# kunalchelani/EdgeGaussians

Measured on AMD Instinct MI355X. Metric: train-step Gaussians*views/sec, higher is better.
Workload: dtype f32; 1 GPU; config2: 100000 Gaussians (5:1 anisotropic, scale 0.004, opacity U(0.05,0.9)), 50 views @512x512, real poses of scan 00004926 (intrinsics 800->512); synthetic wireframe edge maps, loss whole/bg_edge_ratio 4:1; n_gaussians=100000, views=50, width=512, height=512, poses=real poses of scan 00004926 (intrinsics 800->512); synthetic wireframe edge maps, largest_tile_population=2957, gaussian_row_order=morton, binning=segmented, steps_per_native_enqueue=50, forward_mode=chained (exact transmittance stop resolved inside the forward kernel), parallelism=single GPU

## Files before the change

edgegaussians_amd/build.py:

```python
from __future__ import annotations

import os
import shutil
import subprocess
import sys
from concurrent.futures import ThreadPoolExecutor

HERE = os.path.dirname(os.path.abspath(__file__))
CSRC = os.path.join(HERE, "csrc")
LIB = os.path.join(HERE, "libedgegs.so")
OBJ = os.path.join(HERE, "csrc", "_obj")
SOURCES = ["project.hip", "binning.hip", "composite.hip", "composite_wide.hip", "composite_wave.hip", "densify.hip", "knn.hip", "step.hip", "dp.hip", "operator.hip", "backward_fused.hip", "cams.hip", "edges.hip", "sh.hip", "packed.hip", "viewmat_grad.hip", "tiles.hip", "functional.hip", "indices.hip", "adam_sparse.hip", "strategy.hip"]
FLAGS = ["--offload-arch=gfx950", "-O3", "-std=c++17", "-fPIC", "-munsafe-fp-atomics", "-fno-slp-vectorize",
         "-Wall", "-Wno-unused-function"]
FLAGS += os.environ.get("EG_EXTRA_HIPCC_FLAGS", "").split()


def _hipcc() -> str:
    for c in (os.environ.get("HIPCC"), shutil.which("hipcc"), "/opt/rocm/bin/hipcc"):
        if c and os.path.exists(c):
            return c
    raise RuntimeError("hipcc not found: libedgegs.so cannot be built")


STAMP = os.path.join(OBJ, "flags.txt")


def _stale() -> bool:
    if not os.path.exists(LIB):
        return True
    if not os.path.exists(STAMP) or open(STAMP).read() != " ".join(FLAGS):
        return True
    t = os.path.getmtime(LIB)
    deps = [os.path.join(CSRC, f) for f in SOURCES + ["common.h", "composite.h", "project_dev.h", "footprint_dev.h", "wide_dev.h"]]
    deps.append(os.path.join(HERE, "..", "include", "edgegs.h"))
    return any(os.path.getmtime(d) > t for d in deps)


def build(force: bool = False, verbose: bool = True) -> str:
    if not force and not _stale():
        return LIB
    hipcc = _hipcc()
    os.makedirs(OBJ, exist_ok=True)

    def compile_one(src: str) -> str:
        obj = os.path.join(OBJ, src.replace(".hip", ".o"))
        cmd = [hipcc, *FLAGS, "-c", os.path.join(CSRC, src), "-o", obj]
        r = subprocess.run(cmd, capture_output=True, text=True)
        if r.returncode != 0:
            raise RuntimeError(f"hipcc failed on {src}:\n{r.stderr}")
        if verbose and r.stderr.strip():
            print(r.stderr, file=sys.stderr)
        return obj

    with ThreadPoolExecutor(max_workers=len(SOURCES)) as ex:
        objs = list(ex.map(compile_one, SOURCES))
    tmp = LIB + ".tmp"
    r = subprocess.run([hipcc, "--offload-arch=gfx950", "-shared", "-fPIC", *objs, "-ldl", "-o", tmp],
                       capture_output=True, text=True)
    if r.returncode != 0:
        raise RuntimeError(f"link failed:\n{r.stderr}")
    os.replace(tmp, LIB)
    with open(STAMP, "w") as f:
        f.write(" ".join(FLAGS))
    if verbose:
        print(f"built {LIB}")
    return LIB


if __name__ == "__main__":
    build(force="--force" in sys.argv)
```

edgegaussians_amd/csrc/backward_fused.hip:

```cpp
#include "common.h"
#include "footprint_dev.h"
#include "project_dev.h"

namespace eg {

constexpr int kBFWaves = 8;
constexpr int kBFGauss = 8 * kBFWaves;
constexpr int kBFTouched = 512;
static_assert(kBFTouched + 1 <= 8 * kBFWaves * 12, "the touched list reuses the footprint sizes' storage");

struct FusedBwdArgs {
  float *means, *quats, *scales, *opacities;
  const float *viewmat, *K, *next_viewmat, *next_K;
  int N, width, height;
  float eps2d;
  uint32_t flags;
  float4 *splat;
  const StopRec *gtstop;
  float *g2d;
  float *absgrads, *am, *av;
  AdamK hyper;
  int *cursor; int seg_cap; unsigned long long *keys;
  float *loss_part, *loss_out;
};

struct TailLds {
  int *hist, *base, *touched, *ntouched;
};
#ifdef EG_BF_PROF
#define EG_BF_STAMP2(k_)                                                           \
  do {                                                                             \
    if (prof_rec) {                                                                \
      asm volatile("s_waitcnt vmcnt(0) lgkmcnt(0)" ::: "memory");                  \
      const unsigned long long t_ = __builtin_amdgcn_s_memrealtime();              \
      if (lane == 0) prof_rec[k_] = t_;                                            \
    }                                                                              \
  } while (0)
#else
#define EG_BF_STAMP2(k_) do {} while (0)
#endif
__device__ __forceinline__ void gaussian_tail(const FusedBwdArgs &a, const int g, const int lane, Raw raw,
                                              float (&mm)[11], float (&vv)[11], const float4 ga, const float4 gb,
                                              const TailLds lds, unsigned long long *prof_rec) {
  const int width = a.width, height = a.height, N = a.N;
  const int tw = (width + kTile - 1) / kTile, th = (height + kTile - 1) / kTile, T = tw * th;
  const float4 *splat = a.splat;
  int *s_hist = lds.hist, *s_base = lds.base, *s_touched = lds.touched;
  int &s_ntouched = *lds.ntouched;
  const bool alive = g < N;
  if (alive) {
    raw = load_raw(a.means, a.quats, a.scales, a.opacities, g);
    const int radius = __float_as_int(splat[2 * g + 1].w);
    const size_t oM = 0, oS = 3 * (size_t)N, oQ = 6 * (size_t)N, oO = 10 * (size_t)N;
    const Cam cam = load_cam(a.viewmat, a.K);
    Grads gr;
#pragma unroll
    for (int k = 0; k < 3; ++k) gr.mean[k] = gr.scale[k] = 0.f;
#pragma unroll
    for (int k = 0; k < 4; ++k) gr.quat[k] = 0.f;
    gr.opac = 0.f;
    if (radius > 0) {
      const float ag = a.absgrads ? a.absgrads[g] : 0.f;
      Fwd f;
      forward_geom(cam, raw, width, height, -3.0e38f, 3.0e38f, a.eps2d, a.flags, f);
      backward_geom(cam, f, a.eps2d, a.flags, ga, gb, false, 0.f, 0.f, gr);
      if (a.absgrads) a.absgrads[g] = ag + sqrtf(ga.z * ga.z + ga.w * ga.w);
    }
    EG_BF_STAMP2(3);
#pragma unroll
    for (int k = 0; k < 3; ++k) {
      mm[k] = a.am[oM + 3 * g + k]; vv[k] = a.av[oM + 3 * g + k];
      mm[3 + k] = a.am[oS + 3 * g + k]; vv[3 + k] = a.av[oS + 3 * g + k];
    }
#pragma unroll
    for (int k = 0; k < 4; ++k) { mm[6 + k] = a.am[oQ + 4 * g + k]; vv[6 + k] = a.av[oQ + 4 * g + k]; }
    mm[10] = a.am[oO + g]; vv[10] = a.av[oO + g];
#pragma unroll
    for (int k = 0; k < 3; ++k) {
      adam1(raw.m[k], gr.mean[k], mm[k], vv[k], 0, a.hyper);
      a.means[3 * g + k] = raw.m[k]; a.am[oM + 3 * g + k] = mm[k]; a.av[oM + 3 * g + k] = vv[k];
    }
#pragma unroll
    for (int k = 0; k < 3; ++k) {
      adam1(raw.s[k], gr.scale[k], mm[3 + k], vv[3 + k], 1, a.hyper);
      a.scales[3 * g + k] = raw.s[k]; a.am[oS + 3 * g + k] = mm[3 + k]; a.av[oS + 3 * g + k] = vv[3 + k];
    }
#pragma unroll
    for (int k = 0; k < 4; ++k) {
      adam1(raw.q[k], gr.quat[k], mm[6 + k], vv[6 + k], 2, a.hyper);
      a.quats[4 * g + k] = raw.q[k]; a.am[oQ + 4 * g + k] = mm[6 + k]; a.av[oQ + 4 * g + k] = vv[6 + k];
    }
    adam1(raw.o, gr.opac, mm[10], vv[10], 3, a.hyper);
    a.opacities[g] = raw.o; a.am[oO + g] = mm[10]; a.av[oO + g] = vv[10];
  }

  EG_BF_STAMP2(4);
  const Cam ncam = load_cam(a.next_viewmat, a.next_K);
  Fwd f;
  int radius = 0;
  if (alive && forward_geom(ncam, raw, width, height, 0.01f, 1e10f, 0.3f, a.flags, f))
    radius = radius_of(f, width, height, 0.f);
  const bool aa = a.flags & EG_FLAG_ANTIALIASED;
  float4 s0 = make_float4(0.f, 0.f, 0.f, 0.f), s1 = s0;
  if (radius > 0) {
    s0 = make_float4(f.u, f.v, f.a, f.b);
    s1 = make_float4(f.c, aa ? f.o * f.comp : f.o, f.z, __int_as_float(radius));
  }
  if (alive) {
    a.splat[2 * g] = s0;
    a.splat[2 * g + 1] = s1;
  }
  int x0 = 0, y0 = 0, x1 = 0, y1 = 0;
  if (radius > 0) tile_box_tight(s0.x, s0.y, radius, s0.z, s0.w, s1.x, s1.y, tw, th, x0, y0, x1, y1);
  const int bw = x1 - x0;
  const bool small_box = (y1 - y0) * bw <= 32;
  unsigned mask = 0u;
  {
    int bit = 0;
    for (int ty = y0; ty < y1; ++ty)
      for (int tx = x0; tx < x1; ++tx, ++bit) {
        if (!splat_hits_tile(s0.x, s0.y, s0.z, s0.w, s1.x, s1.y, tx, ty)) continue;
        if (small_box) mask |= 1u << bit;
        const int t = ty * tw + tx;
        if (atomicAdd(&s_hist[t], 1) == 0) {
          const int idx = atomicAdd(&s_ntouched, 1);
          if (idx < kBFTouched) s_touched[idx] = t;
        }
      }
  }
  EG_BF_STAMP2(5);
  __builtin_amdgcn_fence(__ATOMIC_RELEASE, "wavefront");
  __builtin_amdgcn_wave_barrier();
  __builtin_amdgcn_fence(__ATOMIC_ACQUIRE, "wavefront");
  const int nt = s_ntouched;
  if (nt <= kBFTouched) {
    for (int i = lane; i < nt; i += 64) {
      const int t = s_touched[i];
      const int c = s_hist[t];
      s_base[t] = atomicAdd(&a.cursor[t], c);
      s_hist[t] = 0;
    }
  } else {
    for (int t = lane; t < T; t += 64) {
      const int c = s_hist[t];
      if (c) { s_base[t] = atomicAdd(&a.cursor[t], c); s_hist[t] = 0; }
    }
  }
  __builtin_amdgcn_fence(__ATOMIC_RELEASE, "wavefront");
  __builtin_amdgcn_wave_barrier();
  __builtin_amdgcn_fence(__ATOMIC_ACQUIRE, "wavefront");
  EG_BF_STAMP2(6);
  const unsigned long long key = ((unsigned long long)(unsigned)__float_as_int(s1.z) << 32) | (unsigned)g;
  for (int ty = y0; ty < y1; ++ty)
    for (int tx = x0; tx < x1; ++tx) {
      const bool hit = small_box ? ((mask >> ((ty - y0) * bw + (tx - x0))) & 1u) != 0u
                                 : splat_hits_tile(s0.x, s0.y, s0.z, s0.w, s1.x, s1.y, tx, ty);
      if (!hit) continue;
      const int t = ty * tw + tx;
      const int slot = s_base[t] + atomicAdd(&s_hist[t], 1);
      if (slot < a.seg_cap) a.keys[(size_t)t * a.seg_cap + slot] = key;
    }
  EG_BF_STAMP2(7);
}

__global__ void __launch_bounds__(64 * kBFWaves) __attribute__((amdgpu_waves_per_eu(4, 4)))
gaussian_bwd_fused_kernel(const FusedBwdArgs a) {
  extern __shared__ __attribute__((aligned(16))) int s_dyn[];
  __shared__ __attribute__((aligned(16))) int s_walk[kBFGauss * 12];
  __shared__ __attribute__((aligned(16))) float s_g2d[kBFGauss * 8];
  float *red = (float *)s_dyn;
  int *s_touched = s_walk;
  int &s_ntouched = s_walk[kBFTouched];
  const int width = a.width, height = a.height, N = a.N;
  const int tw = (width + kTile - 1) / kTile, th = (height + kTile - 1) / kTile, T = tw * th;
  int *s_hist = s_dyn, *s_base = s_dyn + T;
  const int lane = threadIdx.x & 63, wv = threadIdx.x >> 6;
  const float4 *splat = a.splat;
#ifdef EG_BF_PROF
  unsigned long long *prof_rec = (unsigned long long *)(a.g2d + 8 * (size_t)a.N) + (size_t)blockIdx.x * 16;
#define EG_BF_STAMP(k_)                                                            \
  do {                                                                             \
    if (a.g2d && wv == 0) {                                                        \
      asm volatile("s_waitcnt vmcnt(0) lgkmcnt(0)" ::: "memory");                  \
      const unsigned long long t_ = __builtin_amdgcn_s_memrealtime();              \
      if (lane == 0) prof_rec[k_] = t_;                                            \
    }                                                                              \
  } while (0)
#else
#define EG_BF_STAMP(k_) do {} while (0)
#endif
  EG_BF_STAMP(0);
  const int g2 = blockIdx.x * kBFGauss + lane;
  Raw raw = {};
  float mm[11], vv[11];
#pragma unroll
  for (int k = 0; k < 11; ++k) mm[k] = vv[k] = 0.f;

  if (a.loss_part && blockIdx.x == 0 && wv == 1) {
    float v = a.loss_part[lane];
    if (v != 0.f) a.loss_part[lane] = 0.f;
    v = wave_sum_dpp_f(v);
    if (lane == 63 && v != 0.f) unsafeAtomicAdd(a.loss_out, v);
  }
  const int gbase = blockIdx.x * kBFGauss + wv * 8;
  if (threadIdx.x < kBFGauss) {
    const int hg = blockIdx.x * kBFGauss + (int)threadIdx.x;
    Walk w = walk_of(make_float4(0.f, 0.f, 0.f, 0.f), make_float4(0.f, 0.f, 0.f, 0.f), width, height);
    if (hg < N) w = walk_of(splat[2 * hg], splat[2 * hg + 1], width, height);
    int4 *dst = (int4 *)&s_walk[12 * threadIdx.x];
    dst[0] = make_int4(w.i0, w.fh, w.pw, w.jlo);
    dst[1] = make_int4(w.jhi, w.cells, __float_as_int(w.thr), __float_as_int(w.xoff));
    dst[2] = make_int4(__float_as_int(w.shear), 0, 0, 0);
  }
  __syncthreads();
  if (gbase < N) {
    const __amdgpu_buffer_rsrc_t rec_rsrc =
        __builtin_amdgcn_make_buffer_rsrc((void *)a.gtstop, 0, width * height * (int)sizeof(StopRec), 0x00020000);
    Walk h;
    {
      const int4 *src = (const int4 *)&s_walk[12 * (wv * 8 + (lane >> 3))];
      const int4 p = src[0], q = src[1];
      h.i0 = p.x; h.fh = p.y; h.pw = p.z; h.jlo = p.w; h.jhi = q.x; h.cells = q.y;
      h.thr = __int_as_float(q.z); h.xoff = __int_as_float(q.w); h.shear = __int_as_float(src[2].x);
    }
    int total = h.cells, live = h.cells > 0 ? 1 : 0;
#pragma unroll
    for (int d = 8; d < 64; d <<= 1) {
      total += __shfl_xor(total, d, 64);
      live += __shfl_xor(live, d, 64);
    }
    int h_n = 0, h_first = 0;
    Moments m = {0.f, 0.f, 0.f, 0.f, 0.f, 0.f, 0.f, 0.f};
    float4 s0 = make_float4(0.f, 0.f, 0.f, 0.f), s1 = s0;
    if (total > 0) {
      const float share = (float)(64 - live) * (1.f - 1e-5f) * __builtin_amdgcn_rcpf((float)total);
      h_n = h.cells > 0 ? 1 + (int)((float)h.cells * share) : 0;
      int incl = h_n + (h.cells > 0 ? 1 << 16 : 0);
#pragma unroll
      for (int d = 8; d < 64; d <<= 1) {
        const int up = __shfl_up(incl, d, 64);
        if (lane >= d) incl += up;
      }
      const int slack = 64 - (__builtin_amdgcn_readlane(incl, 63) & 0xffff);
      const int rank = (incl >> 16) - (h.cells > 0 ? 1 : 0);
      h_first = (incl & 0xffff) - h_n + min(rank, slack);
      if (h.cells > 0 && rank < slack) ++h_n;
      int k = 0;
#pragma unroll
      for (int q = 1; q < 8; ++q) k += lane >= __builtin_amdgcn_readlane(h_first, 8 * q);
      const int src = 8 * k;
      const int n = max(__shfl(h_n, src, 64), 1);
      const int r = lane - __shfl(h_first, src, 64);
      const int g = min(gbase + k, N - 1);
      const int cells = r < n ? __shfl(h.cells, src, 64) : 0;
      s0 = splat[2 * g];
      s1 = splat[2 * g + 1];
      const int4 *wk = (const int4 *)&s_walk[12 * (wv * 8 + k)];
      const int4 p = wk[0], q = wk[1];
      const float shear_k = __int_as_float(wk[2].x);
      footprint_walk(s0, s1, g, r, n, p.x, cells > 0 ? p.y : 0, max(p.z, 1), p.w, q.x, __int_as_float(q.z),
                     __int_as_float(q.w), shear_k, width, rec_rsrc, m);
    }
    float *mine = red + wv * 256 + lane * 4;
    const int comp = lane & 7;
    float sum = 0.f;
    *(float4 *)mine = make_float4(s0.z * m.w_x + s0.w * m.w_y, s0.w * m.w_x + s1.x * m.w_y, (2.f / kLog2e) * m.abs_x,
                                  (2.f / kLog2e) * m.abs_y);
    __builtin_amdgcn_fence(__ATOMIC_RELEASE, "wavefront");
    __builtin_amdgcn_wave_barrier();
    __builtin_amdgcn_fence(__ATOMIC_ACQUIRE, "wavefront");
    if (comp < 4)
      for (int t = 0; t < h_n; ++t) sum += red[wv * 256 + (h_first + t) * 4 + comp];
    __builtin_amdgcn_fence(__ATOMIC_RELEASE, "wavefront");
    __builtin_amdgcn_wave_barrier();
    __builtin_amdgcn_fence(__ATOMIC_ACQUIRE, "wavefront");
    *(float4 *)mine = make_float4(0.5f * m.w_xx, m.w_xy, 0.5f * m.w_yy, m.v_o);
    __builtin_amdgcn_fence(__ATOMIC_RELEASE, "wavefront");
    __builtin_amdgcn_wave_barrier();
    __builtin_amdgcn_fence(__ATOMIC_ACQUIRE, "wavefront");
    if (comp >= 4)
      for (int t = 0; t < h_n; ++t) sum += red[wv * 256 + (h_first + t) * 4 + comp - 4];
    s_g2d[wv * 64 + lane] = sum;
#ifndef EG_BF_PROF
    if (a.g2d && gbase + (lane >> 3) < N) a.g2d[(size_t)gbase * 8 + lane] = sum;
#endif
  }
  EG_BF_STAMP(1);
  __syncthreads();
  if (wv != 0) return;
  EG_BF_STAMP(2);
  for (int t = lane; t < T; t += 64) s_hist[t] = 0;
  if (lane == 0) s_ntouched = 0;

  {
    const float4 ga = *(const float4 *)&s_g2d[8 * lane], gb = *(const float4 *)&s_g2d[8 * lane + 4];
    const TailLds lds = {s_hist, s_base, s_touched, &s_ntouched};
#ifdef EG_BF_PROF
    unsigned long long *pr = a.g2d ? prof_rec : nullptr;
#else
    unsigned long long *pr = nullptr;
#endif
    gaussian_tail(a, g2, lane, raw, mm, vv, ga, gb, lds, pr);
  }
}

int launch_gaussian_bwd_fused(float *means, float *quats, float *scales, float *opacities, const float *viewmat, const float *K,
                          const float *next_viewmat, const float *next_K, int32_t N, int32_t width, int32_t height,
                          float eps2d, uint32_t flags, float *splat, const float *gtstop, float *g2d, float *absgrads,
                          float *m, float *v, const eg_adam_hyper &hyper, int32_t *tile_cursor, int32_t seg_cap,
                          uint64_t *keys, void *workspace, int64_t max_items, float *loss_out, hipStream_t st) {
  const int T = cdiv(width, kTile) * cdiv(height, kTile);
  if (T > kPrefixHereMaxTiles) {
    set_error("backward_fused: tile grids of <= %d tiles only", kPrefixHereMaxTiles);
    return EG_ERR_ARG;
  }
  if ((int64_t)width * height * (int64_t)sizeof(StopRec) >= (int64_t)kOutOfImage) {
    set_error("backward_fused: image above 2^31 / 12 pixels");
    return EG_ERR_ARG;
  }
  FusedBwdArgs a;
  a.means = means; a.quats = quats; a.scales = scales; a.opacities = opacities;
  a.viewmat = viewmat; a.K = K; a.next_viewmat = next_viewmat; a.next_K = next_K;
  a.N = N; a.width = width; a.height = height; a.eps2d = eps2d; a.flags = flags;
  a.splat = (float4 *)splat; a.gtstop = (const StopRec *)gtstop; a.g2d = g2d;
  a.absgrads = absgrads; a.am = m; a.av = v; a.hyper = make_adamk(hyper);
  a.cursor = tile_cursor; a.seg_cap = seg_cap; a.keys = (unsigned long long *)keys;
  a.loss_part = nullptr; a.loss_out = loss_out;
  if (workspace && loss_out) a.loss_part = carve_workspace(workspace, max_items, T).loss_part;
  gaussian_bwd_fused_kernel<<<cdiv((int64_t)N, kBFGauss), 64 * kBFWaves, sizeof(int) * max(2 * T, kBFWaves * 256), st>>>(a);
  timing_mark(kMarkFootprint, st);
  return check_launch("backward_fused");
}

}
```

edgegaussians_amd/csrc/composite.hip:

```cpp
#include <cstdlib>

#include "common.h"
#include "composite.h"

namespace eg {


struct ModeArgs {
  const float *bg;
  float *v_depths;
  int N;
  int colors_per_camera;
};

__device__ __forceinline__ int camera_list_base(const int *__restrict__ offsets, int T, int c) {
  int base = 0;
  for (int k = 0; k < c; ++k) base += offsets[(size_t)k * (T + 1) + T];
  return base;
}

template <int CH, bool UNIT, bool DEPTH = false, bool BG = false>
__global__ void __launch_bounds__(256)
composite_fwd_kernel(const float4 *__restrict__ splat, const float *__restrict__ colors,
                     const int *__restrict__ offsets, const int *__restrict__ flat, int width, int height,
// ... 569 lines not shown
}

template <int CH>
__global__ void __launch_bounds__(256)
composite_combine_fwd_kernel(const TileTable tt_, const int *__restrict__ flat, int width, int height, int tw,
                             const SliceWs ws_, float *__restrict__ render, float *__restrict__ alphas,
                             int *__restrict__ last_ids, const float *__restrict__ gt, const float *__restrict__ wmap,
                             float loss_scale, float *__restrict__ vpix, float *__restrict__ loss_out,
                             StopRec *__restrict__ gtstop, const Batch bt, int rewalk_skipped) {
  __shared__ float sRed[4];
  const int bv = blockIdx.y;
  const TileTable tt = view_of(tt_, bt, bv);
  const SliceWs ws = view_of(ws_, bt, bv);
  flat += bv * bt.keys;
  if (render) render += bv * bt.pixels * CH;
  if (alphas) alphas += bv * bt.pixels;
  if (last_ids) last_ids += bv * bt.pixels;
  if (vpix) vpix += bv * bt.pixels;
  if (gtstop) gtstop += bv * bt.pixels;
  if (bt.gt[0]) { gt = bt.gt[bv]; wmap = bt.wmap[bv]; }
  const int tile = blockIdx.x, tid = threadIdx.x;
  const int i0 = tt.item_first[tile], ns = tt.item_end[tile] - i0;
  if (ns <= 1) return;
  const int ty = tile / tw, tx = tile - ty * tw;
  int di, dj;
  quad_pixel(tid, di, dj);
  const int i = ty * kTile + di, j = tx * kTile + dj;
  const bool inside = (i < height) && (j < width);
  const bool has_loss = wmap != nullptr;
  const float w_p = (has_loss && inside) ? wmap[i * width + j] : 0.f;
  const float gt_p = (has_loss && inside) ? gt[i * width + j] : 0.f;
  combine_tail<CH, false>(tile, tid, i0, ns, inside, i * width + j, 1.f, 0, -1, ws, flat, render, alphas, last_ids,
                          has_loss, gt_p, w_p, loss_scale, vpix, loss_out, gtstop, sRed, rewalk_skipped != 0);
}

template <int CH>
__global__ void __launch_bounds__(256)
composite_rewalk_fwd_kernel(const float4 *__restrict__ splat, const TileTable tt_,
                            const int *__restrict__ flat, int width, int height, int tw, int th, const SliceWs ws_,
                            float *__restrict__ render, float *__restrict__ alphas, int *__restrict__ last_ids,
                            const float *__restrict__ gt, const float *__restrict__ wmap, float loss_scale,
                            float *__restrict__ vpix, float *__restrict__ loss_out, StopRec *__restrict__ gtstop,
                            const Batch bt) {
  __shared__ QuadLists ql;
  __shared__ float sRed[4];
  const int bv = blockIdx.y;
  const TileTable tt = view_of(tt_, bt, bv);
  const SliceWs ws = view_of(ws_, bt, bv);
  flat += bv * bt.keys; splat += bv * bt.splat4;
  if (render) render += bv * bt.pixels * CH;
  if (alphas) alphas += bv * bt.pixels;
  if (last_ids) last_ids += bv * bt.pixels;
  if (vpix) vpix += bv * bt.pixels;
  if (gtstop) gtstop += bv * bt.pixels;
  if (bt.gt[0]) { gt = bt.gt[bv]; wmap = bt.wmap[bv]; }
  const int tid = threadIdx.x, wv = tid >> 6;
  int di, dj;
  quad_pixel(tid, di, dj);
  const int n_list = ws.ctl[0];
  if ((int)blockIdx.x >= n_list) return;
  for (int k = blockIdx.x; k < n_list; k += gridDim.x) {
  __syncthreads();
  const int2 it = ws.rewalk[k];
  const int b = it.x, tile = it.y;
  const int ty = tile / tw, tx = tile - ty * tw;
  const int i = ty * kTile + di, j = tx * kTile + dj;
  const float px = (float)j + 0.5f, py = (float)i + 0.5f;
  const v2f px2 = {px, px}, py2 = {py, py};
  const int ib = tt.item_first[tile];
  const int s0 = b - ib, ns = tt.item_end[tile] - ib;
  const StopInfo si = ws.stopinfo[(size_t)tile * kTilePix + tid];
  const bool mine = si.slice == s0;
  float T = si.T;
  int last = si.last;
  bool found = false;
  for (int s = s0; s < ns; ++s) {
    if (!__syncthreads_or(mine && !found)) break;
    const int start = tt.start[tile] + s * kSlice, end = min(tt.end[tile], start + kSlice);
    float4 g0 = make_float4(0.f, 0.f, 0.f, 0.f), rB = g0;
    bool hitq[4] = {false, false, false, false};
    if (start + tid < end) {
      const int g = flat[start + tid];
      g0 = splat[2 * g];
      const float4 g1 = splat[2 * g + 1];
      rB = make_float4(g1.x, g1.y, __logf(255.f * g1.y) + kThrMargin, __int_as_float(tid));
      const int m = ws.sliceQ[(size_t)(ib + s) * kSlice + tid];
#pragma unroll
      for (int q = 0; q < 4; ++q) hitq[q] = (m >> q) & 1;
    }
    const int n_mine = build_quad_lists(ql, hitq, g0, rB, tid);
    const float4 *lX = ql.X[wv], *lC = ql.C[wv], *lD = ql.D[wv], *lE = ql.E[wv];
    bool live = mine && !found;
    int lastpos = -1;
    for (int t = 0; t < n_mine && __ballot(live) != 0ull; t += 4) {
      float4 X[2], Cq[2], D[2], E[2];
#pragma unroll
      for (int u = 0; u < 2; ++u) {
        X[u] = lX[(t >> 1) + u]; Cq[u] = lC[(t >> 1) + u]; D[u] = lD[(t >> 1) + u]; E[u] = lE[(t >> 1) + u];
      }
#pragma unroll
      for (int u = 0; u < 2; ++u) {
        const PairEval ev = eval_pair(X[u], Cq[u], D[u], E[u], px2, py2);
        {
          const float nT = T * (1.f - ev.a0);
          const bool hit = live & ev.k0, stop = hit & (nT <= kTStop), upd = hit & !stop;
          T = upd ? nT : T;
          lastpos = upd ? t + 2 * u : lastpos;
          found = found | stop;
          live = live & !stop;
        }
        {
          const float nT = T * (1.f - ev.a1);
          const bool hit = live & ev.k1, stop = hit & (nT <= kTStop), upd = hit & !stop;
          T = upd ? nT : T;
          lastpos = upd ? t + 2 * u + 1 : lastpos;
          found = found | stop;
          live = live & !stop;
        }
      }
    }
    if (lastpos >= 0) last = start + __float_as_int(((const float *)&lE[lastpos >> 1])[2 + (lastpos & 1)]);
  }
  float l = 0.f;
  if (mine)
    l = finalize_pixel<CH>(i * width + j, T, last, found, flat, render, alphas, last_ids, wmap != nullptr,
                           wmap ? gt[i * width + j] : 0.f, wmap ? wmap[i * width + j] : 0.f, loss_scale, vpix, gtstop,
                           splat);
  if (wmap && loss_out) block_loss_add(l, sRed, loss_out);
  if (tid == 0) ws.item_flags[b] = 0;
  }
  if (tid == 0) {
    const int P = min((int)gridDim.x, n_list), grp = blockIdx.x & 63;
    const int members = (P - grp + 63) >> 6;
    if (atomicAdd(&ws.exit_grp[grp * 16], 1) == members - 1) {
      atomicExch(&ws.exit_grp[grp * 16], 0);
      if (atomicAdd(&ws.ctl[1], 1) == min(P, 64) - 1) {
        ws.ctl[2] = max(ws.ctl[2], n_list);
        atomicExch(&ws.ctl[0], 0);
        atomicExch(&ws.ctl[1], 0);
      }
    }
  }
}


}
#include "footprint_dev.h"
namespace eg {

__global__ void __launch_bounds__(256) __attribute__((amdgpu_waves_per_eu(8, 8)))
footprint_bwd_kernel(const float4 *__restrict__ splat, int N, int width, int height,
                     const StopRec *__restrict__ gtstop, float *__restrict__ g2d, const Batch bt,
                     float *__restrict__ loss_part, float *__restrict__ loss_out) {
  __shared__ float red[4][64 * 8];
  splat += blockIdx.y * bt.splat4; gtstop += blockIdx.y * bt.pixels; g2d += blockIdx.y * bt.splat4 * 4;
  const int lane = threadIdx.x & 63, wv = threadIdx.x >> 6;
  if (loss_part && blockIdx.x == 0 && wv == 0) {
    float *lp = (float *)((char *)loss_part + blockIdx.y * bt.ws_bytes);
    float v = lp[lane];
    if (v != 0.f) lp[lane] = 0.f;
    v = wave_sum_dpp_f(v);
    if (lane == 63 && v != 0.f) unsafeAtomicAdd(loss_out, v);
  }
  const int wave = blockIdx.x * 4 + wv;
  const int gbase = wave * 8;
  __shared__ __attribute__((aligned(16))) int s_walk[32][12];
  if (threadIdx.x < 32) {
    const int hg = blockIdx.x * 32 + (int)threadIdx.x;
    Walk w = walk_of(make_float4(0.f, 0.f, 0.f, 0.f), make_float4(0.f, 0.f, 0.f, 0.f), width, height);
    if (hg < N) w = walk_of(splat[2 * hg], splat[2 * hg + 1], width, height);
    int4 *dst = (int4 *)s_walk[threadIdx.x];
    dst[0] = make_int4(w.i0, w.fh, w.pw, w.jlo);
    dst[1] = make_int4(w.jhi, w.cells, __float_as_int(w.thr), __float_as_int(w.xoff));
    dst[2] = make_int4(__float_as_int(w.shear), 0, 0, 0);
  }
  __syncthreads();
  if (gbase >= N) return;
  const __amdgpu_buffer_rsrc_t rec_rsrc =
      __builtin_amdgcn_make_buffer_rsrc((void *)gtstop, 0, width * height * (int)sizeof(StopRec), 0x00020000);

  Walk h;
  {
    const int4 *src = (const int4 *)s_walk[wv * 8 + (lane >> 3)];
    const int4 a = src[0], b = src[1];
    h.i0 = a.x; h.fh = a.y; h.pw = a.z; h.jlo = a.w; h.jhi = b.x; h.cells = b.y;
    h.thr = __int_as_float(b.z); h.xoff = __int_as_float(b.w); h.shear = __int_as_float(src[2].x);
  }
  int total = h.cells, live = h.cells > 0 ? 1 : 0;
#pragma unroll
  for (int d = 8; d < 64; d <<= 1) {
    total += __shfl_xor(total, d, 64);
    live += __shfl_xor(live, d, 64);
  }
  int h_n = 0, h_first = 0;
  Moments m = {0.f, 0.f, 0.f, 0.f, 0.f, 0.f, 0.f, 0.f};
  float4 s0 = make_float4(0.f, 0.f, 0.f, 0.f), s1 = s0;
  if (total > 0) {
    const float share = (float)(64 - live) * (1.f - 1e-5f) * __builtin_amdgcn_rcpf((float)total);
    h_n = h.cells > 0 ? 1 + (int)((float)h.cells * share) : 0;
    int incl = h_n + (h.cells > 0 ? 1 << 16 : 0);
#pragma unroll
    for (int d = 8; d < 64; d <<= 1) {
      const int up = __shfl_up(incl, d, 64);
      if (lane >= d) incl += up;
    }
    const int slack = 64 - (__builtin_amdgcn_readlane(incl, 63) & 0xffff);
    const int rank = (incl >> 16) - (h.cells > 0 ? 1 : 0);
    h_first = (incl & 0xffff) - h_n + min(rank, slack);
    if (h.cells > 0 && rank < slack) ++h_n;
    int k = 0;
#pragma unroll
    for (int q = 1; q < 8; ++q) k += lane >= __builtin_amdgcn_readlane(h_first, 8 * q);
    const int src = 8 * k;
    const int n = max(__shfl(h_n, src, 64), 1);
    const int r = lane - __shfl(h_first, src, 64);
    const int g = min(gbase + k, N - 1);
    const int cells = r < n ? __shfl(h.cells, src, 64) : 0;
    s0 = splat[2 * g];
    s1 = splat[2 * g + 1];
    {
      const int4 *wk = (const int4 *)s_walk[wv * 8 + k];
      const int4 a = wk[0], b = wk[1];
      const float shear_k = __int_as_float(wk[2].x);
      footprint_walk(s0, s1, g, r, n, a.x, cells > 0 ? a.y : 0, max(a.z, 1), a.w, b.x, __int_as_float(b.z),
                     __int_as_float(b.w), shear_k, width, rec_rsrc, m);
    }
  }
  float *mine = &red[wv][lane * 8];
  *(float4 *)mine = make_float4(s0.z * m.w_x + s0.w * m.w_y, s0.w * m.w_x + s1.x * m.w_y, (2.f / kLog2e) * m.abs_x,
                                (2.f / kLog2e) * m.abs_y);
  *(float4 *)(mine + 4) = make_float4(0.5f * m.w_xx, m.w_xy, 0.5f * m.w_yy, m.v_o);
  __builtin_amdgcn_fence(__ATOMIC_RELEASE, "wavefront");
  __builtin_amdgcn_wave_barrier();
  __builtin_amdgcn_fence(__ATOMIC_ACQUIRE, "wavefront");
  const int comp = lane & 7;
  float sum = 0.f;
  for (int t = 0; t < h_n; ++t) sum += red[wv][(h_first + t) * 8 + comp];
  if (gbase + (lane >> 3) < N) g2d[(size_t)gbase * 8 + lane] = sum;
}

__device__ __forceinline__ float wave_sum(float v) {
#pragma unroll
  for (int d = 32; d >= 1; d >>= 1) v += __shfl_xor(v, d, 64);
  return v;
}

template <int CH, bool DEPTH = false, bool BG = false>
__global__ void __launch_bounds__(256)
composite_bwd_colors_kernel(const float4 *__restrict__ splat, const float *__restrict__ colors,
                            const int *__restrict__ offsets, const int *__restrict__ flat, int width,
                            int height, int tw, int th, const float *__restrict__ alphas,
                            const int *__restrict__ last_ids, const float *__restrict__ v_render,
                            const float *__restrict__ v_alphas, float *__restrict__ g2d,
                            float *__restrict__ v_colors, const ModeArgs ma) {
  constexpr bool kModes = DEPTH || BG;
  constexpr int NC = CH + (DEPTH ? 1 : 0);
  constexpr int CA = CH > 0 ? CH : 1;
  static_assert(NC >= 1, "nothing to composite");
  __shared__ float4 sA[kTilePix];
  __shared__ float4 sB[kTilePix];
  __shared__ float sC[kTilePix * CA];
  __shared__ int sG[kTilePix];

  if constexpr (kModes) {
    const int c = blockIdx.y, T = tw * th;
    const size_t hw = (size_t)width * height, n = (size_t)ma.N;
    flat += camera_list_base(offsets, T, c);
    offsets += (size_t)c * (T + 1);
    splat += 2 * n * c;
    if (ma.colors_per_camera) colors += n * CH * c;
    alphas += hw * c;
    last_ids += hw * c;
    v_render += hw * NC * c;
    if (v_alphas) v_alphas += hw * c;
    g2d += 8 * n * c;
    if (v_colors) v_colors += n * CH * c;
  }
  const int tile = xcd_tile(blockIdx.x, tw * th);
  const int start = offsets[tile], end = offsets[tile + 1];
  if (end <= start) return;
  const int tid = threadIdx.x, lane = tid & 63;
  const int ty = tile / tw, tx = tile - ty * tw;
  const int i = ty * kTile + (tid >> 4), j = tx * kTile + (tid & 15);
  const bool inside = (i < height) && (j < width);
  const float px = (float)j + 0.5f, py = (float)i + 0.5f;
  const int p = inside ? i * width + j : 0;

  const float T_final = inside ? 1.f - alphas[p] : 1.f;
  float T = T_final;
  float buffer[CA], vr[CA];
#pragma unroll
  for (int k = 0; k < CH; ++k) { buffer[k] = 0.f; vr[k] = inside ? v_render[(size_t)p * NC + k] : 0.f; }
  float buffer_d = 0.f, vr_d = 0.f;
  if constexpr (DEPTH) vr_d = inside ? v_render[(size_t)p * NC + CH] : 0.f;
  float bg_vr = 0.f;
  if constexpr (BG) {
#pragma unroll
    for (int k = 0; k < CH; ++k) bg_vr += ma.bg[(size_t)blockIdx.y * CH + k] * vr[k];
  }
  const float va_pix = (inside && v_alphas) ? v_alphas[p] : 0.f;
  const int bin_final = (inside && alphas[p] > 0.f) ? last_ids[p] : -1;
  int wave_last = bin_final;
#pragma unroll
  for (int d = 32; d >= 1; d >>= 1) wave_last = max(wave_last, __shfl_xor(wave_last, d, 64));

  const int n_batches = (end - start + kTilePix - 1) / kTilePix;
  for (int b = 0; b < n_batches; ++b) {
    __syncthreads();
    const int batch_end = end - 1 - kTilePix * b;
    const int size = min(kTilePix, batch_end + 1 - start);
    const int idx = batch_end - tid;
    if (idx >= start) {
      const int g = flat[idx];
      const float4 s0 = splat[2 * g], s1 = splat[2 * g + 1];
      sG[tid] = g;
      sA[tid] = s0;
      sB[tid] = make_float4(s1.x, s1.y, DEPTH ? s1.z : 0.f, 0.f);
#pragma unroll
      for (int k = 0; k < CH; ++k) sC[tid * CH + k] = colors ? colors[(size_t)g * CH + k] : 1.f;
    }
    __syncthreads();
    for (int t = max(0, batch_end - wave_last); t < size; ++t) {
      bool valid = inside && (batch_end - t <= bin_final);
      const float4 A = sA[t], B = sB[t];
      const float dx = A.x - px, dy = A.y - py;
      float vis = 0.f, alpha = 0.f;
      if (valid) {
        const float sigma = 0.5f * (A.z * dx * dx + B.x * dy * dy) + A.w * dx * dy;
        vis = __expf(-sigma);
        alpha = fminf(kAlphaMax, B.y * vis);
        if (sigma < 0.f || alpha < kAlphaMin) valid = false;
      }
      if (!__any(valid)) continue;
      float r_rgb[CA];
#pragma unroll
      for (int k = 0; k < CH; ++k) r_rgb[k] = 0.f;
      float r_d = 0.f;
      float gx = 0.f, gy = 0.f, ga = 0.f, gb = 0.f, gc = 0.f, go = 0.f;
      if (valid) {
        const float ra = 1.f / (1.f - alpha);
        T *= ra;
        const float fac = alpha * T;
        float v_alpha = 0.f;
#pragma unroll
        for (int k = 0; k < CH; ++k) {
          r_rgb[k] = fac * vr[k];
          v_alpha += (sC[t * CH + k] * T - buffer[k] * ra) * vr[k];
        }
        if constexpr (DEPTH) {
          r_d = fac * vr_d;
          v_alpha += (B.z * T - buffer_d * ra) * vr_d;
        }
        v_alpha += T_final * ra * va_pix;
        if constexpr (BG) v_alpha += -T_final * ra * bg_vr;
        if (B.y * vis <= kAlphaMax) {
          const float v_sigma = -B.y * vis * v_alpha;
          gx = v_sigma * (A.z * dx + A.w * dy);
          gy = v_sigma * (A.w * dx + B.x * dy);
          ga = 0.5f * v_sigma * dx * dx;
          gb = v_sigma * dx * dy;
          gc = 0.5f * v_sigma * dy * dy;
          go = vis * v_alpha;
        }
#pragma unroll
        for (int k = 0; k < CH; ++k) buffer[k] += sC[t * CH + k] * fac;
        if constexpr (DEPTH) buffer_d += B.z * fac;
      }
      const float agx = wave_sum(fabsf(gx)), agy = wave_sum(fabsf(gy));
      gx = wave_sum(gx); gy = wave_sum(gy);
      ga = wave_sum(ga); gb = wave_sum(gb); gc = wave_sum(gc); go = wave_sum(go);
#pragma unroll
      for (int k = 0; k < CH; ++k) r_rgb[k] = wave_sum(r_rgb[k]);
      if constexpr (DEPTH) r_d = wave_sum(r_d);
      if (lane == 0) {
        const int g = sG[t];
        float *dst = g2d + (size_t)g * 8;
        unsafeAtomicAdd(dst + 0, gx);
        unsafeAtomicAdd(dst + 1, gy);
        unsafeAtomicAdd(dst + 2, agx);
        unsafeAtomicAdd(dst + 3, agy);
        unsafeAtomicAdd(dst + 4, ga);
        unsafeAtomicAdd(dst + 5, gb);
        unsafeAtomicAdd(dst + 6, gc);
        unsafeAtomicAdd(dst + 7, go);
        if (v_colors) {
#pragma unroll
          for (int k = 0; k < CH; ++k) unsafeAtomicAdd(v_colors + (size_t)g * CH + k, r_rgb[k]);
        }
        if constexpr (DEPTH) unsafeAtomicAdd(ma.v_depths + (size_t)blockIdx.y * ma.N + g, r_d);
      }
// ... 271 lines not shown
```

edgegaussians_amd/csrc/footprint_dev.h:

```cpp
#pragma once
#include "composite.h"

namespace eg {

struct Walk {
  int i0, fh;
  int pw;
  int jlo, jhi;
  int cells;
  float thr;
  float xoff, shear;
};

__device__ __forceinline__ Walk walk_of(const float4 s0, const float4 s1, int width, int height) {
  Walk w;
  w.i0 = w.fh = w.pw = w.jlo = w.cells = 0;
  w.jhi = -1;
  w.thr = w.xoff = w.shear = 0.f;
  const int radius = __float_as_int(s1.w);
  const float thr = 0.693147180559945f * __builtin_amdgcn_logf(255.f * s1.y) + kThrMargin;
  const float det = s0.z * s1.x - s0.w * s0.w;
  if (radius <= 0 || !(thr > 0.f) || !(det > 0.f) || !(s0.z > 0.f)) return w;
  const int tw = (width + kTile - 1) / kTile, th = (height + kTile - 1) / kTile;
  int x0, y0, x1, y1;
  tile_box(s0.x, s0.y, radius, tw, th, x0, y0, x1, y1);
  const float k = 2.f * thr * __builtin_amdgcn_rcpf(det);
  const float ex = __builtin_amdgcn_sqrtf(k * s1.x) * 1.001f + 0.01f;
  const float ey = __builtin_amdgcn_sqrtf(k * s0.z) * 1.001f + 0.01f;
  const int j0 = max(x0 * kTile, (int)ceilf(s0.x - ex - 0.5f));
  const int j1 = min(min(x1 * kTile, width) - 1, (int)floorf(s0.x + ex - 0.5f));
  const int i0 = max(y0 * kTile, (int)ceilf(s0.y - ey - 0.5f));
  const int i1 = min(min(y1 * kTile, height) - 1, (int)floorf(s0.y + ey - 0.5f));
  const int fw = j1 - j0 + 1, fh = i1 - i0 + 1;
  if (fw <= 0 || fh <= 0) return w;
  const float inv_a = __builtin_amdgcn_rcpf(s0.z);
  const float hw = __builtin_amdgcn_sqrtf(2.f * thr * inv_a) * 1.001f + 0.01f;
  const int pw = (int)(2.f * hw) + 1;
  w.i0 = i0; w.fh = fh; w.jlo = j0; w.jhi = j1; w.thr = thr;
  if (pw < fw) {
    w.pw = pw; w.shear = s0.w * inv_a; w.xoff = s0.x - hw - 0.5f;
  } else {
    w.pw = fw; w.shear = 0.f; w.xoff = (float)j0;
  }
  w.cells = w.pw * fh;
  return w;
}

struct Moments {
  float w_x, w_y, w_xx, w_xy, w_yy, abs_x, abs_y, v_o;
};

constexpr unsigned kOutOfImage = 0x80000000u;
typedef unsigned u32x3 __attribute__((ext_vector_type(3)));
struct Pair {
  u32x3 rec0, rec1;
  float dx, dy;
};

struct Quad {
  float A, B, C;
  float thr2;
  float o;
  bool high_o;
};
constexpr float kLog2e = 1.44269504088896341f;

__device__ __forceinline__ void footprint_cell(const Quad qd, unsigned g, unsigned dg, const u32x3 rec, float s2, float hx,
                                               float hy, float dx, float dy, Moments &m) {
  const float gT = __uint_as_float(rec.x);
  const bool in = __float_as_uint(s2) <= __float_as_uint(qd.thr2);
  bool counts = rec.z > dg;
  const bool tie = rec.z == dg;
  if (__builtin_amdgcn_ballot_w64(tie) != 0ull) {
    asm volatile("" ::: "memory");
    counts |= tie & (rec.y >= g);
  }
  if (!(gT != 0.f && in && counts)) return;
  const float vis = __builtin_amdgcn_exp2f(-s2);
  const float araw = qd.o * vis;
  bool ok = araw >= kAlphaMin;
  if (qd.high_o) {
    asm volatile("" ::: "memory");
    ok &= araw <= kAlphaMax;
  }
  const float v_alpha = ok ? gT * __builtin_amdgcn_rcpf(1.f - araw) : 0.f;
  m.v_o += vis * v_alpha;
  const float w = -araw * v_alpha;
  const float wx = w * dx, wy = w * dy;
  m.w_x += wx; m.w_y += wy;
  m.w_xx += wx * dx; m.w_xy += wx * dy; m.w_yy += wy * dy;
  m.abs_x = fmaf(fabsf(w), fabsf(hx), m.abs_x);
  m.abs_y = fmaf(fabsf(w), fabsf(hy), m.abs_y);
}

__device__ __forceinline__ void footprint_visit(const Quad qd, unsigned g, unsigned dg, const Pair c, Moments &m) {
  const float dx = c.dx, dy = c.dy;
  const float hx = fmaf(qd.A, dx, qd.B * dy);
  const float hy = fmaf(qd.C, dy, qd.B * dx);
  const float s2 = fmaf(dx, hx, dy * hy);
  const float dx1 = dx - 1.f, hx1 = hx - qd.A, hy1 = hy - qd.B;
  const float s21 = fmaf(dx1, hx1, dy * hy1);
  footprint_cell(qd, g, dg, c.rec0, s2, hx, hy, dx, dy, m);
  footprint_cell(qd, g, dg, c.rec1, s21, hx1, hy1, dx1, dy, m);
}

__device__ __forceinline__ void footprint_walk(const float4 s0, const float4 s1, int g, int r, int n, int i0, int fh,
                                               int pw, int jlo, int jhi, float thr, float xoff,
                                               float shear, int width, const __amdgpu_buffer_rsrc_t gtstop, Moments &m) {
  const int ppr = (pw + 1) >> 1;
  const float inv_ppr = __builtin_amdgcn_rcpf((float)ppr);
  auto divmod = [&](int q, int &qi, int &qj) {
    qi = (int)(((float)q + 0.5f) * inv_ppr);
    qj = q - __mul24(qi, ppr);
    if (qj < 0) { qj += ppr; --qi; }
    if (qj >= ppr) { qj -= ppr; ++qi; }
  };
  const int width12 = width * (int)sizeof(StopRec);
  const float xc = s0.x - 0.5f, yc = s0.y - 0.5f;
  auto fetch = [&](int i, int cp, int live1) -> Pair {
    Pair p;
    p.dy = yc - (float)i;
    const int j = (int)ceilf(xoff + shear * p.dy) + 2 * cp;
    const int t1 = j - jlo, t2 = jhi - j;
    const unsigned bad0 = (unsigned)(t1 | t2 | live1) & kOutOfImage;
    const unsigned bad1 = (unsigned)((t1 + 1) | (t2 - 1) | live1) & kOutOfImage;
    const unsigned base = (unsigned)(__mul24(i, width12) + __mul24(j, 12));
    p.rec0 = __builtin_amdgcn_raw_buffer_load_b96(gtstop, (int)(bad0 | base), 0, 0);
    p.rec1 = __builtin_amdgcn_raw_buffer_load_b96(gtstop, (int)(bad1 | (base + 12u)), 0, 0);
    p.dx = xc - (float)j;
    return p;
  };
  const unsigned ug = (unsigned)g, dg = (unsigned)__float_as_int(s1.z);
  const Quad qd = {0.5f * kLog2e * s0.z, 0.5f * kLog2e * s0.w, 0.5f * kLog2e * s1.x, kLog2e * thr, s1.y,
                   __builtin_amdgcn_ballot_w64(s1.y > kAlphaMax) != 0ull};
  int di, dc;
  divmod(n, di, dc);
  int ia, ca;
  divmod(r, ia, ca);
  ia += i0;
  int left = __mul24(fh, ppr) - r;
  auto advance = [&]() {
    left -= n;
    const int t = ca + dc - ppr, sm = t >> 31;
    ca = t + (ppr & sm);
    ia += di + 1 + sm;
  };
  Pair p0 = fetch(ia, ca, left - 1);
  while (left > 0) {
    advance();
    const Pair p1 = fetch(ia, ca, left - 1);
    footprint_visit(qd, ug, dg, p0, m);
    if (left <= 0) break;
    advance();
    p0 = fetch(ia, ca, left - 1);
    footprint_visit(qd, ug, dg, p1, m);
  }
}

}
```

Before: 1.306 billion Gaussians*views/s.

## Precompute lane deal per Gaussian group in the sizing pass and stage splats in LDS

Moves the per-wave lane-allocation (deal) computation out of the shuffle-heavy scan in the footprint backward kernels. The 32/64 sizing threads now compute each group's lane count and first lane with a scalar loop and store them in LDS. They also stage the splat records in an inbox, so walking lanes read splat data and deal info from LDS instead of global memory and cross-lane shuffles. The final per-Gaussian reduction becomes a 4-way unrolled fold. This removes DPP/shuffle latency and duplicate global splat loads. In exchange it adds a serial 8-iteration loop per sizing thread and slightly more LDS.

Result: faster. 1.321 billion Gaussians*views/s, median of 6 (+1.2%).

```diff
diff --git a/edgegaussians_amd/build.py b/edgegaussians_amd/build.py
--- a/edgegaussians_amd/build.py
+++ b/edgegaussians_amd/build.py
@@ -32,7 +32,7 @@
     if not os.path.exists(STAMP) or open(STAMP).read() != " ".join(FLAGS):
         return True
     t = os.path.getmtime(LIB)
-    deps = [os.path.join(CSRC, f) for f in SOURCES + ["common.h", "composite.h", "project_dev.h", "footprint_dev.h", "wide_dev.h"]]
+    deps = [os.path.join(CSRC, f) for f in SOURCES + ["common.h", "composite.h", "project_dev.h", "footprint_dev.h", "deal_rule.h", "wide_dev.h"]]
     deps.append(os.path.join(HERE, "..", "include", "edgegs.h"))
     return any(os.path.getmtime(d) > t for d in deps)
 
diff --git a/edgegaussians_amd/csrc/backward_fused.hip b/edgegaussians_amd/csrc/backward_fused.hip
--- a/edgegaussians_amd/csrc/backward_fused.hip
+++ b/edgegaussians_amd/csrc/backward_fused.hip
@@ -166,7 +166,7 @@
 __global__ void __launch_bounds__(64 * kBFWaves) __attribute__((amdgpu_waves_per_eu(4, 4)))
 gaussian_bwd_fused_kernel(const FusedBwdArgs a) {
   extern __shared__ __attribute__((aligned(16))) int s_dyn[];
-  __shared__ __attribute__((aligned(16))) int s_walk[kBFGauss * 12];
+  __shared__ __attribute__((aligned(16))) int s_walk[kBFGauss * kHomeRow];
   __shared__ __attribute__((aligned(16))) float s_g2d[kBFGauss * 8];
   float *red = (float *)s_dyn;
   int *s_touched = s_walk;
@@ -204,73 +204,28 @@
   }
   const int gbase = blockIdx.x * kBFGauss + wv * 8;
   if (threadIdx.x < kBFGauss) {
-    const int hg = blockIdx.x * kBFGauss + (int)threadIdx.x;
-    Walk w = walk_of(make_float4(0.f, 0.f, 0.f, 0.f), make_float4(0.f, 0.f, 0.f, 0.f), width, height);
-    if (hg < N) w = walk_of(splat[2 * hg], splat[2 * hg + 1], width, height);
-    int4 *dst = (int4 *)&s_walk[12 * threadIdx.x];
-    dst[0] = make_int4(w.i0, w.fh, w.pw, w.jlo);
-    dst[1] = make_int4(w.jhi, w.cells, __float_as_int(w.thr), __float_as_int(w.xoff));
-    dst[2] = make_int4(__float_as_int(w.shear), 0, 0, 0);
+    const int t = (int)threadIdx.x;
+    footprint_size_and_deal(splat, blockIdx.x * kBFGauss + t, N, width, height, t, &s_walk[kHomeRow * t],
+                            &s_walk[kHomeRow * (t & ~7)], red + (t >> 3) * 256);
   }
   __syncthreads();
   if (gbase < N) {
     const __amdgpu_buffer_rsrc_t rec_rsrc =
         __builtin_amdgcn_make_buffer_rsrc((void *)a.gtstop, 0, width * height * (int)sizeof(StopRec), 0x00020000);
-    Walk h;
-    {
-      const int4 *src = (const int4 *)&s_walk[12 * (wv * 8 + (lane >> 3))];
-      const int4 p = src[0], q = src[1];
-      h.i0 = p.x; h.fh = p.y; h.pw = p.z; h.jlo = p.w; h.jhi = q.x; h.cells = q.y;
-      h.thr = __int_as_float(q.z); h.xoff = __int_as_float(q.w); h.shear = __int_as_float(src[2].x);
-    }
-    int total = h.cells, live = h.cells > 0 ? 1 : 0;
-#pragma unroll
-    for (int d = 8; d < 64; d <<= 1) {
-      total += __shfl_xor(total, d, 64);
-      live += __shfl_xor(live, d, 64);
-    }
-    int h_n = 0, h_first = 0;
+    float *slice = red + wv * 256;
     Moments m = {0.f, 0.f, 0.f, 0.f, 0.f, 0.f, 0.f, 0.f};
-    float4 s0 = make_float4(0.f, 0.f, 0.f, 0.f), s1 = s0;
-    if (total > 0) {
-      const float share = (float)(64 - live) * (1.f - 1e-5f) * __builtin_amdgcn_rcpf((float)total);
-      h_n = h.cells > 0 ? 1 + (int)((float)h.cells * share) : 0;
-      int incl = h_n + (h.cells > 0 ? 1 << 16 : 0);
-#pragma unroll
-      for (int d = 8; d < 64; d <<= 1) {
-        const int up = __shfl_up(incl, d, 64);
-        if (lane >= d) incl += up;
-      }
-      const int slack = 64 - (__builtin_amdgcn_readlane(incl, 63) & 0xffff);
-      const int rank = (incl >> 16) - (h.cells > 0 ? 1 : 0);
-      h_first = (incl & 0xffff) - h_n + min(rank, slack);
-      if (h.cells > 0 && rank < slack) ++h_n;
-      int k = 0;
-#pragma unroll
-      for (int q = 1; q < 8; ++q) k += lane >= __builtin_amdgcn_readlane(h_first, 8 * q);
-      const int src = 8 * k;
-      const int n = max(__shfl(h_n, src, 64), 1);
-      const int r = lane - __shfl(h_first, src, 64);
-      const int g = min(gbase + k, N - 1);
-      const int cells = r < n ? __shfl(h.cells, src, 64) : 0;
-      s0 = splat[2 * g];
-      s1 = splat[2 * g + 1];
-      const int4 *wk = (const int4 *)&s_walk[12 * (wv * 8 + k)];
-      const int4 p = wk[0], q = wk[1];
-      const float shear_k = __int_as_float(wk[2].x);
-      footprint_walk(s0, s1, g, r, n, p.x, cells > 0 ? p.y : 0, max(p.z, 1), p.w, q.x, __int_as_float(q.z),
-                     __int_as_float(q.w), shear_k, width, rec_rsrc, m);
-    }
-    float *mine = red + wv * 256 + lane * 4;
+    float4 s0, s1;
+    footprint_home_walk(&s_walk[kHomeRow * wv * 8], slice, lane, gbase, N, width, rec_rsrc, s0, s1, m);
+    float *mine = slice + lane * 4;
     const int comp = lane & 7;
+    const int2 nf = *(const int2 *)&s_walk[kHomeRow * (wv * 8 + (lane >> 3)) + 10];
+    const float *theirs = slice + nf.y * 4 + (comp & 3);
     float sum = 0.f;
-    *(float4 *)mine = make_float4(s0.z * m.w_x + s0.w * m.w_y, s0.w * m.w_x + s1.x * m.w_y, (2.f / kLog2e) * m.abs_x,
-                                  (2.f / kLog2e) * m.abs_y);
+    *(float4 *)mine = footprint_partial_means(s0, s1, m);
     __builtin_amdgcn_fence(__ATOMIC_RELEASE, "wavefront");
     __builtin_amdgcn_wave_barrier();
     __builtin_amdgcn_fence(__ATOMIC_ACQUIRE, "wavefront");
-    if (comp < 4)
-      for (int t = 0; t < h_n; ++t) sum += red[wv * 256 + (h_first + t) * 4 + comp];
+    if (comp < 4) sum = footprint_fold<4>(theirs, nf.x);
     __builtin_amdgcn_fence(__ATOMIC_RELEASE, "wavefront");
     __builtin_amdgcn_wave_barrier();
     __builtin_amdgcn_fence(__ATOMIC_ACQUIRE, "wavefront");
@@ -278,8 +233,7 @@
     __builtin_amdgcn_fence(__ATOMIC_RELEASE, "wavefront");
     __builtin_amdgcn_wave_barrier();
     __builtin_amdgcn_fence(__ATOMIC_ACQUIRE, "wavefront");
-    if (comp >= 4)
-      for (int t = 0; t < h_n; ++t) sum += red[wv * 256 + (h_first + t) * 4 + comp - 4];
+    if (comp >= 4) sum = footprint_fold<4>(theirs, nf.x);
     s_g2d[wv * 64 + lane] = sum;
 #ifndef EG_BF_PROF
     if (a.g2d && gbase + (lane >> 3) < N) a.g2d[(size_t)gbase * 8 + lane] = sum;
@@ -327,7 +281,7 @@
   a.cursor = tile_cursor; a.seg_cap = seg_cap; a.keys = (unsigned long long *)keys;
   a.loss_part = nullptr; a.loss_out = loss_out;
   if (workspace && loss_out) a.loss_part = carve_workspace(workspace, max_items, T).loss_part;
-  gaussian_bwd_fused_kernel<<<cdiv((int64_t)N, kBFGauss), 64 * kBFWaves, sizeof(int) * max(2 * T, kBFWaves * 256), st>>>(a);
+  gaussian_bwd_fused_kernel<<<cdiv((int64_t)N, kBFGauss), 64 * kBFWaves, sizeof(int) * max(2 * T, kBFWaves * 256 + kHomeFoldPad * 4), st>>>(a);
   timing_mark(kMarkFootprint, st);
   return check_launch("backward_fused");
 }
diff --git a/edgegaussians_amd/csrc/composite.hip b/edgegaussians_amd/csrc/composite.hip
--- a/edgegaussians_amd/csrc/composite.hip
+++ b/edgegaussians_amd/csrc/composite.hip
@@ -745,7 +745,8 @@
 footprint_bwd_kernel(const float4 *__restrict__ splat, int N, int width, int height,
                      const StopRec *__restrict__ gtstop, float *__restrict__ g2d, const Batch bt,
                      float *__restrict__ loss_part, float *__restrict__ loss_out) {
-  __shared__ float red[4][64 * 8];
+  __shared__ __attribute__((aligned(16))) float red[4 * 64 * 8 + kHomeFoldPad * 8];
+  static_assert(kHomeInbox <= 64 * 8, "a wave's inbox lies in its slice of the exchange");
   splat += blockIdx.y * bt.splat4; gtstop += blockIdx.y * bt.pixels; g2d += blockIdx.y * bt.splat4 * 4;
   const int lane = threadIdx.x & 63, wv = threadIdx.x >> 6;
   if (loss_part && blockIdx.x == 0 && wv == 0) {
@@ -757,78 +758,30 @@
   }
   const int wave = blockIdx.x * 4 + wv;
   const int gbase = wave * 8;
-  __shared__ __attribute__((aligned(16))) int s_walk[32][12];
+  __shared__ __attribute__((aligned(16))) int s_walk[32][kHomeRow];
   if (threadIdx.x < 32) {
-    const int hg = blockIdx.x * 32 + (int)threadIdx.x;
-    Walk w = walk_of(make_float4(0.f, 0.f, 0.f, 0.f), make_float4(0.f, 0.f, 0.f, 0.f), width, height);
-    if (hg < N) w = walk_of(splat[2 * hg], splat[2 * hg + 1], width, height);
-    int4 *dst = (int4 *)s_walk[threadIdx.x];
-    dst[0] = make_int4(w.i0, w.fh, w.pw, w.jlo);
-    dst[1] = make_int4(w.jhi, w.cells, __float_as_int(w.thr), __float_as_int(w.xoff));
-    dst[2] = make_int4(__float_as_int(w.shear), 0, 0, 0);
+    const int t = (int)threadIdx.x;
+    footprint_size_and_deal(splat, blockIdx.x * 32 + t, N, width, height, t, s_walk[t], s_walk[t & ~7],
+                            red + (t >> 3) * 512);
   }
   __syncthreads();
   if (gbase >= N) return;
   const __amdgpu_buffer_rsrc_t rec_rsrc =
       __builtin_amdgcn_make_buffer_rsrc((void *)gtstop, 0, width * height * (int)sizeof(StopRec), 0x00020000);
 
-  Walk h;
-  {
-    const int4 *src = (const int4 *)s_walk[wv * 8 + (lane >> 3)];
-    const int4 a = src[0], b = src[1];
-    h.i0 = a.x; h.fh = a.y; h.pw = a.z; h.jlo = a.w; h.jhi = b.x; h.cells = b.y;
-    h.thr = __int_as_float(b.z); h.xoff = __int_as_float(b.w); h.shear = __int_as_float(src[2].x);
-  }
-  int total = h.cells, live = h.cells > 0 ? 1 : 0;
-#pragma unroll
-  for (int d = 8; d < 64; d <<= 1) {
-    total += __shfl_xor(total, d, 64);
-    live += __shfl_xor(live, d, 64);
-  }
-  int h_n = 0, h_first = 0;
+  float *slice = red + wv * 512;
   Moments m = {0.f, 0.f, 0.f, 0.f, 0.f, 0.f, 0.f, 0.f};
-  float4 s0 = make_float4(0.f, 0.f, 0.f, 0.f), s1 = s0;
-  if (total > 0) {
-    const float share = (float)(64 - live) * (1.f - 1e-5f) * __builtin_amdgcn_rcpf((float)total);
-    h_n = h.cells > 0 ? 1 + (int)((float)h.cells * share) : 0;
-    int incl = h_n + (h.cells > 0 ? 1 << 16 : 0);
-#pragma unroll
-    for (int d = 8; d < 64; d <<= 1) {
-      const int up = __shfl_up(incl, d, 64);
-      if (lane >= d) incl += up;
-    }
-    const int slack = 64 - (__builtin_amdgcn_readlane(incl, 63) & 0xffff);
-    const int rank = (incl >> 16) - (h.cells > 0 ? 1 : 0);
-    h_first = (incl & 0xffff) - h_n + min(rank, slack);
-    if (h.cells > 0 && rank < slack) ++h_n;
-    int k = 0;
-#pragma unroll
-    for (int q = 1; q < 8; ++q) k += lane >= __builtin_amdgcn_readlane(h_first, 8 * q);
-    const int src = 8 * k;
-    const int n = max(__shfl(h_n, src, 64), 1);
-    const int r = lane - __shfl(h_first, src, 64);
-    const int g = min(gbase + k, N - 1);
-    const int cells = r < n ? __shfl(h.cells, src, 64) : 0;
-    s0 = splat[2 * g];
-    s1 = splat[2 * g + 1];
-    {
-      const int4 *wk = (const int4 *)s_walk[wv * 8 + k];
-      const int4 a = wk[0], b = wk[1];
-      const float shear_k = __int_as_float(wk[2].x);
-      footprint_walk(s0, s1, g, r, n, a.x, cells > 0 ? a.y : 0, max(a.z, 1), a.w, b.x, __int_as_float(b.z),
-                     __int_as_float(b.w), shear_k, width, rec_rsrc, m);
-    }
-  }
-  float *mine = &red[wv][lane * 8];
-  *(float4 *)mine = make_float4(s0.z * m.w_x + s0.w * m.w_y, s0.w * m.w_x + s1.x * m.w_y, (2.f / kLog2e) * m.abs_x,
-                                (2.f / kLog2e) * m.abs_y);
+  float4 s0, s1;
+  footprint_home_walk(s_walk[wv * 8], slice, lane, gbase, N, width, rec_rsrc, s0, s1, m);
+  float *mine = slice + lane * 8;
+  *(float4 *)mine = footprint_partial_means(s0, s1, m);
   *(float4 *)(mine + 4) = make_float4(0.5f * m.w_xx, m.w_xy, 0.5f * m.w_yy, m.v_o);
   __builtin_amdgcn_fence(__ATOMIC_RELEASE, "wavefront");
   __builtin_amdgcn_wave_barrier();
   __builtin_amdgcn_fence(__ATOMIC_ACQUIRE, "wavefront");
   const int comp = lane & 7;
-  float sum = 0.f;
-  for (int t = 0; t < h_n; ++t) sum += red[wv][(h_first + t) * 8 + comp];
+  const int2 nf = *(const int2 *)&s_walk[wv * 8 + (lane >> 3)][10];
+  const float sum = footprint_fold<8>(slice + nf.y * 8 + comp, nf.x);
   if (gbase + (lane >> 3) < N) g2d[(size_t)gbase * 8 + lane] = sum;
 }
 
diff --git a/edgegaussians_amd/csrc/deal_rule.h b/edgegaussians_amd/csrc/deal_rule.h
--- /dev/null
+++ b/edgegaussians_amd/csrc/deal_rule.h
@@ -0,0 +1,41 @@
+#pragma once
+
+#if defined(__HIPCC__)
+#define EG_DEAL_HD __host__ __device__ __forceinline__
+#else
+#define EG_DEAL_HD inline
+#endif
+
+namespace eg {
+
+constexpr int kDealLanes = 64, kDealGroups = 8;
+
+struct Deal {
+  int n, first;
+};
+
+EG_DEAL_HD void deal_totals(const int (&cells)[kDealGroups], int &total, int &live) {
+  total = 0; live = 0;
+  for (int j = 0; j < kDealGroups; ++j) {
+    total += cells[j];
+    live += cells[j] > 0 ? 1 : 0;
+  }
+}
+
+EG_DEAL_HD Deal deal_lanes(const int (&cells)[kDealGroups], int live, float inv_total, int i) {
+  const float share = (float)(kDealLanes - live) * (1.f - 1e-5f) * inv_total;
+  int sum = 0, before = 0, rank = 0, mine = 0;
+  for (int j = 0; j < kDealGroups; ++j) {
+    const int nj = cells[j] > 0 ? 1 + (int)((float)cells[j] * share) : 0;
+    if (j < i) { before += nj; rank += cells[j] > 0 ? 1 : 0; }
+    if (j == i) mine = nj;
+    sum += nj;
+  }
+  const int slack = kDealLanes - sum;
+  Deal d;
+  d.first = before + (rank < slack ? rank : slack);
+  d.n = mine + ((mine > 0 && rank < slack) ? 1 : 0);
+  return d;
+}
+
+}
diff --git a/edgegaussians_amd/csrc/footprint_dev.h b/edgegaussians_amd/csrc/footprint_dev.h
--- a/edgegaussians_amd/csrc/footprint_dev.h
+++ b/edgegaussians_amd/csrc/footprint_dev.h
@@ -1,5 +1,6 @@
 #pragma once
 #include "composite.h"
+#include "deal_rule.h"
 
 namespace eg {
 
@@ -157,4 +158,73 @@
   }
 }
 
-}
+constexpr int kHomeRow = 12;
+constexpr int kHomeInbox = 72;
+constexpr int kHomeFoldPad = 3;
+
+__device__ __forceinline__ void footprint_size_and_deal(const float4 *__restrict__ splat, int hg, int N, int width,
+                                                        int height, int t, int *row, const int *rows8, float *inbox) {
+  const int gc = min(hg, N - 1);
+  const float4 s0 = splat[2 * gc], s1 = splat[2 * gc + 1];
+  Walk w = walk_of(make_float4(0.f, 0.f, 0.f, 0.f), make_float4(0.f, 0.f, 0.f, 0.f), width, height);
+  if (hg < N) w = walk_of(s0, s1, width, height);
+  int4 *dst = (int4 *)row;
+  dst[0] = make_int4(w.i0, w.fh, w.pw, w.jlo);
+  dst[1] = make_int4(w.jhi, w.cells, __float_as_int(w.thr), __float_as_int(w.xoff));
+  const int i = t & 7;
+  *(float4 *)(inbox + 8 * i) = s0;
+  *(float4 *)(inbox + 8 * i + 4) = s1;
+  __builtin_amdgcn_fence(__ATOMIC_RELEASE, "wavefront");
+  __builtin_amdgcn_wave_barrier();
+  __builtin_amdgcn_fence(__ATOMIC_ACQUIRE, "wavefront");
+  int cells[kDealGroups];
+#pragma unroll
+  for (int j = 0; j < kDealGroups; ++j) cells[j] = rows8[kHomeRow * j + 5];
+  int total, live;
+  deal_totals(cells, total, live);
+  Deal d = {0, 0};
+  if (total > 0) d = deal_lanes(cells, live, __builtin_amdgcn_rcpf((float)total), i);
+  dst[2] = make_int4(__float_as_int(w.shear), 0, d.n, d.first);
+  inbox[64 + i] = __int_as_float(i == 0 ? total : d.first);
+}
+
+__device__ __forceinline__ void footprint_home_walk(const int *rows8, const float *inbox, int lane, int gbase, int N,
+                                                    int width, const __amdgpu_buffer_rsrc_t rec_rsrc, float4 &s0,
+                                                    float4 &s1, Moments &m) {
+  const float4 f0 = *(const float4 *)(inbox + 64), f1 = *(const float4 *)(inbox + 68);
+  s0 = s1 = make_float4(0.f, 0.f, 0.f, 0.f);
+  if (__float_as_int(f0.x) <= 0) return;
+  const int k = (lane >= __float_as_int(f0.y)) + (lane >= __float_as_int(f0.z)) + (lane >= __float_as_int(f0.w)) +
+                (lane >= __float_as_int(f1.x)) + (lane >= __float_as_int(f1.y)) + (lane >= __float_as_int(f1.z)) +
+                (lane >= __float_as_int(f1.w));
+  const int4 *wk = (const int4 *)(rows8 + kHomeRow * k);
+  const int4 a = wk[0], b = wk[1], c = wk[2];
+  const int n = max(c.z, 1);
+  const int r = lane - c.w;
+  const int g = min(gbase + k, N - 1);
+  const int cells = r < n ? b.y : 0;
+  s0 = *(const float4 *)(inbox + 8 * k);
+  s1 = *(const float4 *)(inbox + 8 * k + 4);
+  footprint_walk(s0, s1, g, r, n, a.x, cells > 0 ? a.y : 0, max(a.z, 1), a.w, b.x, __int_as_float(b.z),
+                 __int_as_float(b.w), __int_as_float(c.x), width, rec_rsrc, m);
+}
+
+__device__ __forceinline__ float4 footprint_partial_means(const float4 s0, const float4 s1, const Moments &m) {
+  return make_float4(fmaf(s0.z, m.w_x, s0.w * m.w_y), fmaf(s1.x, m.w_y, s0.w * m.w_x), (2.f / kLog2e) * m.abs_x,
+                     (2.f / kLog2e) * m.abs_y);
+}
+
+template <int STRIDE>
+__device__ __forceinline__ float footprint_fold(const float *p, int n) {
+  float sum = 0.f;
+  for (int t = 0; t < n; t += 4, p += 4 * STRIDE) {
+    const float v0 = p[0], v1 = p[STRIDE], v2 = p[2 * STRIDE], v3 = p[3 * STRIDE];
+    sum += v0;
+    sum += t + 1 < n ? v1 : 0.f;
+    sum += t + 2 < n ? v2 : 0.f;
+    sum += t + 3 < n ? v3 : 0.f;
+  }
+  return sum;
+}
+
+}
```
